# jimmyshe/liorf

Measured on AMD Instinct MI355X. Metric: LM iterations/sec (64-line scan vs 200k-pt map), higher is better.
Workload: dtype f32; 1 GPU; kitti64: 120000-pt scan vs 200000-pt local surf map, 30 LM iterations per scan (early exit off), one scan per GPU at a time, 8 distinct seeded scans in rotation, map replicated; n_q=120000, n_m=200000, distinct_scans=8, parallelism=scan-per-gpu x1

## Files before the change

### include/liorf_s2m_debug.h

```cpp
#ifndef LIORF_S2M_DEBUG_H
#define LIORF_S2M_DEBUG_H

#include "liorf_s2m.h"

#ifdef __cplusplus
extern "C" {
#endif

int  s2m_debug_device_trig(s2m_handle h, const float* x, size_t n, float* s, float* c, float* a);
int  s2m_debug_deferred(s2m_handle h, int slot);
int  s2m_time_iteration_kernel(s2m_handle h, const float pose[6], int reps, float* ms_per_launch);
int  s2m_time_iterations(s2m_handle h, const float pose[6], int reps, float* ms_per_iter, int cap);

int  s2m_time_loop_launches(s2m_handle h, const float pose[6], int reps, float* us_per_launch);

int  s2m_debug_time_steady(s2m_handle h, const float pose[6], int reps, int solve_prev, float* us_per_launch);

#define S2M_PROF_WORDS 32
int  s2m_debug_wave_profile(s2m_handle h, const float pose[6], int launches, uint64_t* out, size_t cap_waves);

int  s2m_debug_device_hypot(s2m_handle h, const float* x, const float* y, size_t n, float* r);

typedef struct s2m_debug_lm_close_out {
    float   AtA[36], AtB[6];
    int32_t n_sel_last;
    s2m_iter_trace trace;
    float   pose[6];
    float   pose_next[6];
    int32_t iters_run, converged, done, stalled, is_degenerate;
    int32_t n_rows_active;
    float   matP[36];
} s2m_debug_lm_close_out;
int  s2m_debug_lm_close(s2m_handle h, int form, int iter, const double* rows, int n_rows, const float pose0[6],
// ... 20 lines not shown
```

### liorf_amd/csrc/s2m_abi.hip

```cpp
#include <hip/hip_runtime.h>

#include <cfloat>
#include <cmath>
#include <cstdio>
#include <cstdlib>
#include <cstring>
#include <algorithm>
#include <limits>
#include <map>
#include <new>
#include <string>
#include <vector>

#include "s2m_context.hpp"
#include "s2m_kernels.hpp"

using namespace s2m;
using namespace s2m::host;

namespace {

inline uint32_t host_f2ord(float f) { uint32_t u; memcpy(&u, &f, 4); return (u & 0x80000000u) ? ~u : (u | 0x80000000u); }
inline float host_ord2f(uint32_t o) { uint32_t u = (o & 0x80000000u) ? (o & 0x7fffffffu) : ~o; float f; memcpy(&f, &u, 4); return f; }

inline float stamps_ms(const s2m_context* h, int from, int to)
{
    const unsigned long long a = h->reg.h_stamps[from], b = h->reg.h_stamps[to];
    return (b > a && h->reg.wall_clock_khz > 0) ? (float)((double)(b - a) / (double)h->reg.wall_clock_khz) : 0.0f;
}

int ensure_rows(s2m_context* h, int nblocks)
{
    const size_t rows = sizeof(double) * 2 * kAcc * (size_t)nblocks;
    int rc = ensure(h, h->reg.partials, rows + 64 + sizeof(int32_t) * 2 * (size_t)nblocks);
    if (rc) return rc;
    h->hctx.partials = h->reg.partials.as<double>();
    h->hctx.wl_count = reinterpret_cast<int32_t*>(h->reg.partials.as<unsigned char>() + rows);
// ... 229 lines not shown
}

void launch_scan_prep(hipStream_t stream, const PrepTable& t, int nslots)
{
    int npb = 0, nb = 0, ncb = 0;
    for (int k = 0; k < nslots; k++) {
        npb = std::max(npb, (int)t.s[k].npb);
        nb = std::max(nb, (t.s[k].n + 255) / 256);
        ncb = std::max(ncb, (t.s[k].n_chunks + 3) / 4);
    }
    if (npb == 0) return;
    hipLaunchKernelGGL(k_polar_count, dim3(npb, nslots), dim3(kPolarBlock), 0, stream, t);
    hipLaunchKernelGGL(k_polar_prefix, dim3(kPolarCells / 64, nslots), dim3(1024), 0, stream, t);
    hipLaunchKernelGGL(k_polar_scan, dim3(1, nslots), dim3(1024), 0, stream, t);
    hipLaunchKernelGGL(k_scatter_scan, dim3(nb, nslots), dim3(256), 0, stream, t);
    hipLaunchKernelGGL(k_chunk_parts, dim3(ncb, nslots), dim3(256), 0, stream, t);
    hipLaunchKernelGGL(k_chunk_table, dim3(1, nslots), dim3(1024), 0, stream, t);
}

}

int s2m::host::set_scan_impl(s2m_context* h, const void* pts, size_t n, size_t stride, bool on_device)
{
    S2M_HIP(h, hipSetDevice(h->device));
    PrepTable t;
    int rc = scan_slot_prepare(h, pts, n, stride, on_device, &t.s[0]);
    if (rc) return rc;
    if (n == 0) { h->reg.t_set_scan_ms = 0; h->reg.scan_timing_pending = false; return upload_ctx(h); }
    t.s[0].stamps = h->reg.h_stamps + kStampPrep0;
    launch_scan_prep(h->stream, t, 1);
    S2M_HIP(h, hipGetLastError());
    h->reg.scan_timing_pending = true;
    if (!on_device) S2M_HIP(h, hipEventSynchronize(h->reg.ev_up));
    return S2M_OK;
}

namespace {

void fill_state(s2m_context* h, DevState* s, const float pose[6])
{
    memset(s, 0, sizeof(*s));
    memcpy(s->pose, pose, 24);
    memcpy(s->pose2[0], pose, 24);
    host_pose_to_transform(pose, s->T, s->sc);
    s->T_valid = 1;
    memcpy(s->matP, h->reg.persist_matP, sizeof(s->matP));
    s->isDegenerate = h->reg.persist_degenerate;
}

int push_state(s2m_context* h, const float pose[6], unsigned long long* stamp = nullptr)
{
    DevState s;
    fill_state(h, &s, pose);
    if (h->ctx_dirty) {
        hipLaunchKernelGGL(k_set_ctx_state, dim3(1), dim3(64), 0, h->stream, h->reg.dctx.as<DevCtx>(), h->hctx, h->reg.state.as<DevState>(), s,
                           (const int32_t*)h->reg.n_waves.as<int32_t>(), stamp);
        h->ctx_dirty = false;
    } else
        hipLaunchKernelGGL(k_set_state, dim3(1), dim3(64), 0, h->stream, h->reg.state.as<DevState>(), s,
                           (const int32_t*)h->reg.n_waves.as<int32_t>(), stamp);
    S2M_HIP(h, hipGetLastError());
    return S2M_OK;
}

constexpr int kFuseMaxBlocks = 512;
static_assert(sizeof(CtxTable) <= 4096 && sizeof(StateInitTable) <= 4096 && sizeof(PrepTable) <= 4096 && sizeof(SlotTable) <= 4096,
              "kernel arguments are limited to 4 KB");

struct LoopShape {
    SlotTable tbl;
    int nslots = 1;
    int nblocks = 0;
    int table_cap = 0;
    int wpb = kBlock / 64;
    bool batch = false;
    bool split = false;
    bool late = false;
    bool split_auto = false;
    DevState* out = nullptr;
    unsigned long long* stamp = nullptr;
};

LoopShape shape_of(s2m_context* h)
{
    LoopShape sh;
    memset(&sh.tbl, 0, sizeof(sh.tbl));
    sh.tbl.ctx[0] = h->reg.dctx.as<DevCtx>();
    sh.tbl.st[0] = h->reg.state.as<DevState>();
    sh.nslots = 1; sh.nblocks = h->hctx.nblocks; sh.table_cap = h->hctx.table_cap; sh.wpb = h->hctx.wpb;
    sh.batch = h->batch.parent != nullptr && !h->batch.slot_mode;
    sh.split = h->tune.split_mode == 1;
    return sh;
}

template <bool HOOK, int NW, int MINW, int MODE, int CNW>
inline void launch_k(hipStream_t s, const LoopShape& sh, int L, int flags, int grid_x = 0)
{
    hipLaunchKernelGGL((k_register<HOOK, NW, MINW, MODE, CNW>), dim3(grid_x > 0 ? std::min(grid_x, sh.nblocks) : sh.nblocks, sh.nslots), dim3(NW * 64), 0, s,
                       sh.tbl, L, flags);
}

inline void launch_fused(s2m_context* h, const LoopShape& sh, bool hook, int L, int solve_prev)
{
// ... 22 lines not shown
}

inline void launch_certify(s2m_context* h, const LoopShape& sh, int L, int solve_prev, bool fused_loop)
{
    constexpr int NW = kBlock / 64;
    const int fl = solve_prev ? kFlagSolvePrev : 0;
    if (!fused_loop && sh.wpb == NW && h->tune.lean_certify)
        hipLaunchKernelGGL((k_certify_lean<NW, 1, kCertifyLeanWaves>), dim3(sh.nblocks, sh.nslots), dim3(NW * 64), 0, h->stream, sh.tbl, L);
    else if (sh.wpb == kBigWaves) launch_k<false, kBigWaves, kCertifyWavesBig, kCertify, kBigWaves>(h->stream, sh, L, fl);
    else                     launch_k<false, NW, kCertifyWaves, kCertify, NW>(h->stream, sh, L, fl);
}

inline void launch_iteration(s2m_context* h, const LoopShape& sh, int L, int solve_prev, bool fused_loop = true)
{
    if (!sh.split) { launch_fused(h, sh, false, L, solve_prev); return; }
    if (L == 0) { launch_search(h, sh, 0, true); return; }
    launch_certify(h, sh, L, solve_prev, fused_loop);
    launch_search(h, sh, L, false, sh.late);
}

inline void launch_finalize(s2m_context* h, const LoopShape& sh, int L, int mode, bool ends_range = false)
{
    hipLaunchKernelGGL(k_finalize, dim3(1, sh.nslots), dim3(kFinThreads), 0, h->stream, sh.tbl, L, mode,
                       ends_range ? sh.out : (DevState*)nullptr, ends_range ? sh.stamp : (unsigned long long*)nullptr);
}

inline void launch_density(s2m_context* h, const LoopShape& sh)
{
    hipLaunchKernelGGL(k_wave_density, dim3((sh.table_cap + 3) / 4, sh.nslots), dim3(256), 0, h->stream, sh.tbl, h->tune.density_raw);
    hipLaunchKernelGGL(k_chunk_table_density, dim3(1, sh.nslots), dim3(1024), 0, h->stream, sh.tbl);
}

void enqueue_loop(s2m_context* h, const LoopShape& sh_in, hipEvent_t* events, bool coarse = false, int L0 = 0, int L1 = -1)
{
    const int n = h->prm.max_iter;
    if (L1 < 0) L1 = n;
    const bool fuse = h->tune.fuse_solve && sh_in.nblocks * sh_in.nslots <= h->tune.fuse_max_blocks;
    LoopShape sh = sh_in;
    const bool split_late = sh.split_auto && !fuse && sh.wpb == kBlock / 64 && h->tune.lean_certify;
    if (h->tune.density_raw > 0 && L0 == 0) launch_density(h, sh);
    for (int L = L0; L < L1; L++) {
        const int slot = !coarse ? 2 * L : (L == 0 ? 0 : (L == 1 ? 2 : (L == n - 1 ? 6 : 4)));
        const bool open = events && (!coarse || L <= 2 || L == n - 1), close = events && (!coarse || L <= 1 || L >= n - 2);
        if (open) (void)hipEventRecord(events[slot], h->stream);
        sh.split = sh_in.split || (split_late && L >= h->tune.split_from);
        sh.late = !sh_in.split && sh.split;
        launch_iteration(h, sh, L, (fuse && L >= 2 && L != L0) ? 1 : 0, fuse);
        if (close) (void)hipEventRecord(events[slot + 1], h->stream);
        if ((!fuse || L == 0 || L == L1 - 1) && !(sh.late && h->tune.close_in_search)) launch_finalize(h, sh, L, 0, L == L1 - 1);
    }
}

int get_graph(s2m_context* h, int nblocks, int part, hipGraphExec_t* out)
{
    LoopShape sh = shape_of(h);
    sh.out = &h->reg.h_state[1];
    sh.stamp = part == 2 ? nullptr : h->reg.h_stamps + kStampLoop1;
    const long long key = (((long long)h->hctx.table_cap * 4 + part) * 256 + (part ? h->tune.seg_iters : 0)) * 4 + (sh.split ? 1 : 0) + (sh.wpb == kBigWaves ? 2 : 0);
    auto it = h->reg.graphs.find(key);
    if (it != h->reg.graphs.end()) { *out = it->second; return S2M_OK; }
    hipGraph_t graph = nullptr;
    hipGraphExec_t exec = nullptr;
    S2M_HIP(h, hipStreamBeginCapture(h->stream, hipStreamCaptureModeThreadLocal));
    enqueue_loop(h, sh, nullptr, false, part == 2 ? h->tune.seg_iters : 0, part == 1 ? h->tune.seg_iters : -1);
    hipError_t e = hipStreamEndCapture(h->stream, &graph);
    if (e != hipSuccess || !graph) return fail(h, S2M_ERR_HIP, "hipStreamEndCapture", e);
    e = hipGraphInstantiate(&exec, graph, nullptr, nullptr, 0);
    (void)hipGraphDestroy(graph);
    if (e != hipSuccess) return fail(h, S2M_ERR_HIP, "hipGraphInstantiate", e);
    h->reg.graphs[key] = exec;
    *out = exec;
    return S2M_OK;
}

int launch_loop(s2m_context* h, int part = 0)
{
    const int nblocks = h->hctx.nblocks;
    if (h->tune.use_graph) {
        hipGraphExec_t exec = nullptr;
        int rc = get_graph(h, nblocks, part, &exec);
        if (rc == S2M_OK) {
            if (part == 2) S2M_HIP(h, hipEventRecord(h->reg.ev_a2, h->stream));
            S2M_HIP(h, hipGraphLaunch(exec, h->stream));
            if (part == 2) S2M_HIP(h, hipEventRecord(h->reg.ev_b2, h->stream));
            h->hctx.density_pending = 0;
            return S2M_OK;
        }
        h->tune.use_graph = false;
    }
    LoopShape sh = shape_of(h);
    sh.stamp = part == 2 ? nullptr : h->reg.h_stamps + kStampLoop1;
    if (part == 2) S2M_HIP(h, hipEventRecord(h->reg.ev_a2, h->stream));
    enqueue_loop(h, sh, nullptr, false, part == 2 ? h->tune.seg_iters : 0, part == 1 ? h->tune.seg_iters : -1);
    S2M_HIP(h, hipGetLastError());
    if (part == 2) S2M_HIP(h, hipEventRecord(h->reg.ev_b2, h->stream));
    S2M_HIP(h, hipMemcpyAsync(&h->reg.h_state[1], h->reg.state.p, sizeof(DevState) + sizeof(s2m_iter_trace) * h->prm.max_iter, hipMemcpyDeviceToHost, h->stream));
    h->hctx.density_pending = 0;
    return S2M_OK;
}

void params_to_ctx(s2m_context* h, const s2m_params& prm)
{
    h->hctx.gate_f = nextafterf((float)prm.gate_sq, INFINITY);
    h->hctx.gate_r = nextafterf(sqrtf((float)prm.gate_sq), 0.0f);
    h->hctx.gate_sq = prm.gate_sq; h->hctx.plane_tol = prm.plane_tol; h->hctx.weight_scale = prm.weight_scale;
    h->hctx.weight_min = prm.weight_min; h->hctx.conv_deg = prm.conv_deg; h->hctx.conv_cm = prm.conv_cm;
    h->hctx.eig_thresh = prm.eig_thresh; h->hctx.min_corr = prm.min_corr; h->hctx.max_iter = prm.max_iter;
    h->hctx.early_exit = prm.early_exit;
    h->ctx_dirty = true;
}

constexpr size_t kScDesc = (size_t)S2M_SC_NUM_RING * S2M_SC_NUM_SECTOR;

int sc_reserve(s2m_context* h, size_t want)
{
    if (want <= h->sc.cap) return S2M_OK;
    size_t cap = h->sc.cap ? h->sc.cap : 256;
    while (cap < want) cap *= 2;
    struct Part { DevBuf* b; size_t elem; } parts[3] = { { &h->sc.store_desc, sizeof(double) * kScDesc },
                                                         { &h->sc.store_ring, sizeof(float) * S2M_SC_NUM_RING },
// ... 73 lines not shown
    if (hipGetDeviceCount(&count) != hipSuccess || count <= 0 || prm.device_id < 0 || prm.device_id >= count)
        return S2M_ERR_NO_DEVICE;
    if (hipSetDevice(prm.device_id) != hipSuccess) return S2M_ERR_NO_DEVICE;
    hipDeviceProp_t prop;
    if (hipGetDeviceProperties(&prop, prm.device_id) != hipSuccess) return S2M_ERR_NO_DEVICE;
    if (strncmp(prop.gcnArchName, "gfx950", 6) != 0) return S2M_ERR_NO_DEVICE;

    s2m_context* h = new (std::nothrow) s2m_context();
    if (!h) return S2M_ERR_HIP;
    h->prm = prm; h->device = prm.device_id;
    if (const char* e = getenv("S2M_NO_GRAPH")) h->tune.use_graph = !(e[0] == '1');
    if (const char* e = getenv("S2M_NO_FUSE")) h->tune.fuse_solve = !(e[0] == '1');
    if (const char* e = getenv("S2M_DENSITY_RAW")) h->tune.density_raw = atoi(e);
    if (const char* e = getenv("S2M_BIG_BLOCKS")) h->tune.big_blocks = !(e[0] == '0');
    if (const char* e = getenv("S2M_SEGMENT")) h->tune.seg_iters = atoi(e);
    if (const char* e = getenv("S2M_SPLIT")) h->tune.split_mode = atoi(e);
    if (const char* e = getenv("S2M_LOCKSTEP")) h->tune.lockstep = !(e[0] == '0');
    if (const char* e = getenv("S2M_SPLIT_FROM")) h->tune.split_from = std::max(1, atoi(e));
    if (const char* e = getenv("S2M_SEARCH_GRID")) h->tune.search_grid = std::max(1, atoi(e));
    if (const char* e = getenv("S2M_CLOSE_IN_SEARCH")) h->tune.close_in_search = (e[0] == '1');
    if (const char* e = getenv("S2M_BATCH_MINW")) h->tune.batch_minw = atoi(e);
    if (const char* e = getenv("S2M_BATCH_ENTRIES")) h->tune.batch_entries = atoi(e);
    if (const char* e = getenv("S2M_LEAN")) h->tune.lean_certify = !(e[0] == '0');
    h->tune.fuse_max_blocks = kFuseMaxBlocks;
    if (const char* e = getenv("S2M_FUSE_MAX")) h->tune.fuse_max_blocks = atoi(e);

    auto bail = [&](int code) { s2m_destroy(h); return code; };
    if (prm.stream) { h->stream = static_cast<hipStream_t>(prm.stream); h->own_stream = false; }
    else {
        if (hipStreamCreateWithFlags(&h->stream, hipStreamNonBlocking) != hipSuccess) return bail(S2M_ERR_HIP);
        h->own_stream = true;
    }
    if (hipEventCreate(&h->reg.ev_a) != hipSuccess || hipEventCreate(&h->reg.ev_b) != hipSuccess ||
        hipEventCreate(&h->reg.ev_c) != hipSuccess || hipEventCreate(&h->reg.ev_d) != hipSuccess ||
        hipEventCreate(&h->reg.ev_a2) != hipSuccess || hipEventCreate(&h->reg.ev_b2) != hipSuccess ||
        hipEventCreateWithFlags(&h->reg.ev_up, hipEventDisableTiming) != hipSuccess) return bail(S2M_ERR_HIP);
    static_assert(sizeof(DevState) % 8 == 0, "the trace follows the state block");
    if (hipHostMalloc((void**)&h->reg.h_state, sizeof(DevState) * 2 + sizeof(s2m_iter_trace) * kMaxIter) != hipSuccess) return bail(S2M_ERR_HIP);
    h->reg.h_trace = reinterpret_cast<s2m_iter_trace*>(h->reg.h_state + 2);
    if (hipHostMalloc((void**)&h->reg.h_mm, 64) != hipSuccess) return bail(S2M_ERR_HIP);
    if (hipHostMalloc((void**)&h->reg.h_stamps, sizeof(unsigned long long) * kStampCount) != hipSuccess) return bail(S2M_ERR_HIP);
    memset(h->reg.h_stamps, 0, sizeof(unsigned long long) * kStampCount);
    {
        int khz = 0;
        if (hipDeviceGetAttribute(&khz, hipDeviceAttributeWallClockRate, prm.device_id) != hipSuccess || khz <= 0) { khz = 0; (void)hipGetLastError(); }
        h->reg.wall_clock_khz = khz;
// ... 106 lines not shown
    h->reg.pending_skipped = 0;
    if (h->reg.n_m == 0) { h->reg.pending_skipped = 1; return S2M_OK; }
    if ((int)h->reg.n_q <= h->prm.min_feats) { h->reg.pending_skipped = 2; return S2M_OK; }
    int rc;
    if ((rc = push_state(h, pose, h->reg.h_stamps + kStampLoop0))) return rc;
    h->reg.seg_pending = h->prm.early_exit && h->tune.seg_iters > 1 && h->tune.seg_iters < h->prm.max_iter;
    if ((rc = launch_loop(h, h->reg.seg_pending ? 1 : 0))) return rc;
    return S2M_OK;
}

int s2m_optimize_collect(s2m_handle h, float pose[6], const s2m_imu_init* imu, s2m_result* out)
{
    if (!h || !pose) return S2M_ERR_INVALID_ARG;
    if (!h->reg.opt_pending) return fail(h, S2M_ERR_INVALID_ARG, "no optimize launch pending");
    h->reg.opt_pending = false;
    s2m_result r;
    memset(&r, 0, sizeof(r));
    r.skipped = h->reg.pending_skipped;
    h->reg.last_trace_n = 0;
    float t[6];
    memcpy(t, h->reg.pending_pose_in, 24);
    if (!r.skipped) {
        S2M_HIP(h, hipSetDevice(h->device));
        S2M_HIP(h, hipStreamSynchronize(h->stream));
        if (h->batch.parent && !h->batch.slot_mode) h->reg.t_optimize_ms = h->batch.parent->reg.t_optimize_ms;
        else h->reg.t_optimize_ms = stamps_ms(h, kStampLoop0, kStampLoop1);
        if (h->reg.seg_pending && !h->reg.h_state[1].done) {
            int rc2 = launch_loop(h, 2);
            if (rc2) return rc2;
            S2M_HIP(h, hipStreamSynchronize(h->stream));
            float t2 = 0.0f;
            S2M_HIP(h, hipEventElapsedTime(&t2, h->reg.ev_a2, h->reg.ev_b2));
            h->reg.t_optimize_ms += t2;
        }
        h->reg.seg_pending = false;
        const DevState& s = h->reg.h_state[1];
        memcpy(t, s.pose, 24);
        r.iters_run = s.iters_run; r.converged = s.converged; r.is_degenerate = s.isDegenerate;
        r.n_sel_last = s.n_sel_last;
        h->reg.persist_degenerate = s.isDegenerate;
        memcpy(h->reg.persist_matP, s.matP, sizeof(s.matP));
        int n_exec = s.iters_run, stall_at = -1;
        for (int i = 0; i < n_exec && i < kMaxIter; i++) {
            if (stall_at >= 0) { h->reg.last_trace[i] = h->reg.last_trace[stall_at]; continue; }
            h->reg.last_trace[i] = h->reg.h_trace[i];
            if (s.stalled && !h->reg.h_trace[i].stepped) stall_at = i;
        }
        h->reg.last_trace_n = n_exec < kMaxIter ? n_exec : kMaxIter;
        host_transform_update(h->prm, imu, t, r.affine);
    } else {
        host_pose_to_transform(t, r.affine, nullptr);
        r.is_degenerate = h->reg.persist_degenerate;
// ... 565 lines not shown

int s2m_debug_deferred(s2m_handle h, int slot)
{
    if (!h) return S2M_ERR_INVALID_ARG;
    if (slot >= 0) { if (slot >= (int)h->batch.kids.size()) return S2M_ERR_INVALID_ARG; h = h->batch.kids[(size_t)slot]; }
    return h->reg.h_state ? h->reg.h_state[1].deferred_total : 0;
}

int s2m_last_timing(s2m_handle h, float* optimize_ms, float* set_map_ms, float* set_scan_ms)
{
    if (!h) return S2M_ERR_INVALID_ARG;
    if (h->reg.scan_timing_pending) {
        S2M_HIP(h, hipSetDevice(h->device));
        S2M_HIP(h, hipStreamSynchronize(h->stream));
        h->reg.t_set_scan_ms = stamps_ms(h, kStampPrep0, kStampPrep1);
        h->reg.scan_timing_pending = false;
    }
    if (optimize_ms) *optimize_ms = h->reg.t_optimize_ms;
    if (set_map_ms) *set_map_ms = h->reg.t_set_map_ms;
    if (set_scan_ms) *set_scan_ms = h->reg.t_set_scan_ms;
    return S2M_OK;
}

static int time_iterations_impl(s2m_handle h, const float pose[6], int reps, float* ms_mean, float* ms_per_iter)
{
    if (!h || !pose || reps < 1) return S2M_ERR_INVALID_ARG;
    if (!h->reg.have_scan || h->reg.n_m == 0 || h->reg.n_q == 0) return fail(h, S2M_ERR_NO_SCAN, "needs a resident scan and map");
    S2M_HIP(h, hipSetDevice(h->device));
    int rc;
    if ((rc = upload_ctx(h))) return rc;
    const int nit = h->prm.max_iter;
    if (h->reg.iter_events.size() < (size_t)(2 * nit)) {
        const size_t old = h->reg.iter_events.size();
        h->reg.iter_events.resize(2 * nit);
        for (size_t k = old; k < h->reg.iter_events.size(); k++) S2M_HIP(h, hipEventCreate(&h->reg.iter_events[k]));
    }
    std::vector<double> per_iter((size_t)nit, 0.0);
    for (int rep = 0; rep < reps; rep++) {
        S2M_HIP(h, hipMemsetAsync(h->reg.cert.p, 0, sizeof(float4) * h->reg.n_q, h->stream));
        S2M_HIP(h, hipMemsetAsync(h->reg.aux.p, 0, sizeof(int4) * h->reg.n_q, h->stream));
        if ((rc = push_state(h, pose))) return rc;
        enqueue_loop(h, shape_of(h), h->reg.iter_events.data());
        h->hctx.density_pending = 0;
        S2M_HIP(h, hipGetLastError());
        S2M_HIP(h, hipStreamSynchronize(h->stream));
        for (int it = 0; it < nit; it++) {
// ... 183 lines not shown
```

### liorf_amd/csrc/s2m_context.hpp

```cpp
#pragma once
#include <hip/hip_runtime.h>

#include <cstddef>
#include <cstdint>
#include <map>
#include <string>
#include <vector>

#include "s2m_types.h"
#include "s2m_host_math.hpp"
#include "s2m_voxel.hpp"
#include "s2m_icp.hpp"
#include "s2m_project.hpp"
#include "s2m_pose_graph.hpp"

namespace s2m {
namespace host __attribute__((visibility("hidden"))) {

struct DevBuf {
    void*  p = nullptr;
    size_t cap = 0;
    DevBuf() = default;
    DevBuf(const DevBuf&) = delete;
    DevBuf& operator=(const DevBuf&) = delete;
    ~DevBuf() { (void)reset(); }
    template <typename T> T* as() const { return reinterpret_cast<T*>(p); }
    hipError_t reset(void* q = nullptr, size_t bytes = 0)
    {
        const hipError_t e = p ? hipFree(p) : hipSuccess;
        p = q; cap = bytes;
        return e;
    }
    void forget() { p = nullptr; cap = 0; }
};

constexpr size_t kDsStride = 32;

enum { kStampPrep0 = 0, kStampPrep1 = 1, kStampLoop0 = 2, kStampLoop1 = 3, kStampCount = 4 };

}
}

struct __attribute__((visibility("hidden"))) s2m_context {
    using DevBuf = s2m::host::DevBuf;

    s2m_params prm{};
    int device = 0;
    hipStream_t stream = nullptr;
    bool own_stream = false;
    std::string err;
    s2m::DevCtx hctx{};
    bool ctx_dirty = true;

    struct Registration {
        DevBuf raw_map, map_sorted, m_counts, m_cell_start, m_cell_of, m_rank_of;
        DevBuf raw_scan, qx, qy, qz, qperm, npos, front, cert, aux, plane_cache, plane_alt, npos_alt, chunk_parts, chunk_factor, wave_table, n_waves, q_counts, q_cell_start, q_cell_of, q_rank_of, q_block_hist;
        DevBuf block_sums, partials, state, dctx, mm, dbg_idx5, dbg_d2, dbg_flag, dbg_coeff, dbg_clk;
        size_t n_m = 0, n_q = 0;
        bool have_scan = false;

        s2m::DevState* h_state = nullptr;
        s2m_iter_trace* h_trace = nullptr;
        uint32_t* h_mm = nullptr;
        unsigned long long* h_stamps = nullptr;
        int wall_clock_khz = 0;

        int persist_degenerate = 0;
        float persist_matP[36] = { 0 };

        std::map<long long, hipGraphExec_t> graphs;
        std::vector<hipEvent_t> iter_events;
        hipEvent_t ev_a = nullptr, ev_b = nullptr, ev_c = nullptr, ev_d = nullptr, ev_up = nullptr;
        hipEvent_t ev_a2 = nullptr, ev_b2 = nullptr;
        float t_optimize_ms = 0, t_set_map_ms = 0, t_set_scan_ms = 0;
        int base_parts = 1;
        bool seg_pending = false;
        bool opt_pending = false;
        bool scan_timing_pending = false;
        int pending_skipped = 0;
        float pending_pose_in[6] = { 0 };
        s2m_iter_trace last_trace[s2m::kMaxIter];
        int last_trace_n = 0;
    } reg;

    struct Batch {
        s2m_context* parent = nullptr;
        std::vector<s2m_context*> kids;
        std::vector<hipStream_t> branch_streams;
        std::vector<hipEvent_t> branch_events;
        std::vector<hipEvent_t> prep_events;
        std::vector<char> prep_pending;
        hipEvent_t ev_fork = nullptr, ev_prep = nullptr;
        DevBuf kid_states;
        unsigned char* h_kid_states = nullptr;
        bool slot_mode = false;
        bool state_borrowed = false;
        std::map<std::vector<int>, hipGraphExec_t> graphs;
        std::vector<int> live;
        bool seg_pending = false;
        unsigned long long map_epoch = 0;
        unsigned long long adopted_epoch = 0;
    } batch;

    struct Tuning {
        bool use_graph = true;
        bool fuse_solve = true;
        int  fuse_max_blocks = 0;
        int  seg_iters = 8;
        int  split_mode = -1;
        bool tune_env = false;
        bool lean_certify = true;
        int  batch_entries = 1;
        int  batch_minw = 4;
        bool close_in_search = false;
        int  search_grid = 8;
        int  split_from = 8;
        bool lockstep = true;
        bool big_blocks = true;
        int  density_raw = 320;
    } tune;

    struct Voxel {
        DevBuf in, out, frames_xf, scan_ds, map_ds;
        s2m::VoxWorkspace* ws = nullptr;
        size_t scan_ds_n = 0;
        bool have_scan_ds = false;
    } voxel;

    struct ScanContext {
        DevBuf bins, out;
        DevBuf store_desc, store_ring, store_sector, cand;
        size_t n = 0, cap = 0, n_search = 0;
        int    counter = 0;
        double* h_stage = nullptr;
    } sc;

    struct KeyFrames {
        DevBuf pos, frames, tdev;
        std::vector<void*> blocks;
        size_t block_used = 0, block_cap = 0, cap = 0;
        std::vector<float> pose;
// ... 154 lines not shown
```

### liorf_amd/csrc/s2m_kernels.hpp

```cpp
#pragma once
#include <float.h>
#include <math.h>
#include <string.h>
#include "s2m_types.h"

#if defined(__HIPCC__)
#define S2M_HD __host__ __device__
#else
#define S2M_HD
#endif

namespace s2m {

template <typename T> using gptr = __attribute__((address_space(1))) T*;
template <typename T> __device__ __forceinline__ gptr<T> G(T* p) { return (gptr<T>)p; }
typedef float v4f __attribute__((ext_vector_type(4)));
typedef const __attribute__((address_space(4))) DevCtx* CtxP;
__device__ __forceinline__ CtxP ctx_const(const DevCtx* p) { return (CtxP)p; }
__device__ __forceinline__ GridDesc grid_of(CtxP cp)
{
    GridDesc g;
    g.ox = cp->g.ox; g.oy = cp->g.oy; g.oz = cp->g.oz; g.inv_e = cp->g.inv_e; g.e = cp->g.e;
    g.nx = cp->g.nx; g.ny = cp->g.ny; g.nz = cp->g.nz; g.ncells = cp->g.ncells;
    return g;
// ... 1228 lines not shown
    const float mnz = wave_min_f32(fin ? sz : INFINITY), mxz = wave_max_f32(fin ? sz : -INFINITY);
    if (!(mnx <= mxx)) return;
    const GridDesc g = grid_of(cp);
    const auto cell_start = G(cp->cell_start);
    const int bx0 = max(cell_coord(mnx, g.ox, g.inv_e, g.nx) - 1, 0), bx1 = min(cell_coord(mxx, g.ox, g.inv_e, g.nx) + 1, g.nx - 1);
    const int by0 = max(cell_coord(mny, g.oy, g.inv_e, g.ny) - 1, 0), by1 = min(cell_coord(mxy, g.oy, g.inv_e, g.ny) + 1, g.ny - 1);
    const int bz0 = max(cell_coord(mnz, g.oz, g.inv_e, g.nz) - 1, 0), bz1 = min(cell_coord(mxz, g.oz, g.inv_e, g.nz) + 1, g.nz - 1);
    const int nyb = by1 - by0 + 1, nzb = bz1 - bz0 + 1;
    if (nyb * nzb > kRowMax) return;
    int raw = 0;
    for (int r = lane; r < nyb * nzb; r += 64) {
        const int zq = r / nyb;
        const int gcell = ((bz0 + zq) * g.ny + by0 + (r - zq * nyb)) * g.nx;
        raw += cell_start[gcell + bx1 + 1] - cell_start[gcell + bx0];
    }
    raw = __builtin_amdgcn_readlane(wave_incl_scan_i32(raw), 63);
    int f = raw <= raw_limit ? 1 : (raw <= 2 * raw_limit ? 2 : (raw <= 4 * raw_limit ? 4 : 8));
    f = min(f, max(e.y / 8, 1));
    if (lane == 0 && f > 1) atomicMax(&cp->chunk_factor[e.x >> 6], f);
}

#include "s2m_register.hpp"

__device__ __forceinline__ void finalize_record_out(gptr<DevState> st, DevState* out, int max_iter, unsigned long long* stamp)
{
    static_assert(sizeof(DevState) % 4 == 0 && sizeof(s2m_iter_trace) % 4 == 0, "the record is copied word by word");
    if (out) {
        const auto src = (gptr<const uint32_t>)st;
        const auto dst = G(reinterpret_cast<uint32_t*>(out));
        const int nw = (int)((sizeof(DevState) + sizeof(s2m_iter_trace) * (size_t)max_iter) / 4);
        for (int k = threadIdx.x; k < nw; k += kFinThreads) dst[k] = src[k];
    }
    if (stamp) {
        __syncthreads();
        if (threadIdx.x == 0) *stamp = wall_clock64();
    }
}

__global__ __launch_bounds__(kFinThreads) void k_finalize(const SlotTable tbl, int iter, int mode, DevState* out, unsigned long long* stamp)
{
    const CtxP cp = ctx_const(tbl.ctx[blockIdx.y]);
    const auto st = G(tbl.st[blockIdx.y]);
    const int done0 = st->done, degen0 = st->isDegenerate;
    const int nb_act = (st->n_waves + cp->wpb - 1) / cp->wpb;
    float pose0[6];
#pragma unroll
    for (int k = 0; k < 6; k++) pose0[k] = st->pose2[iter & 1][k];
    if (mode == 0 && done0) { finalize_record_out(st, out, cp->max_iter, stamp); return; }
    __shared__ LmShared sh;
    __shared__ float s_out[8];
    if (mode == 0 && threadIdx.x == 0 && cp->wl_count) { cp->wl_count[0] = 0; cp->wl_count[1] = 0; }
    float pose[6];
    const bool ended = lm_close_iteration<kFinThreads, true>(cp, st, nb_act, iter, true, mode == 1, pose0, degen0, sh, s_out, pose);
    if (mode == 0 && !ended && threadIdx.x < 64) {
        float T[12], sc6[6];
        build_transform(pose, (int)threadIdx.x, T, sc6);
        if (threadIdx.x == 0 && !st->stalled) {
#pragma unroll
            for (int k = 0; k < 12; k++) st->T[k] = T[k];
#pragma unroll
            for (int k = 0; k < 6; k++) st->sc[k] = sc6[k];
            st->T_valid = 1;
        }
    }
    if (out || stamp) {
        __syncthreads();
        finalize_record_out(st, out, cp->max_iter, stamp);
    }
}

__global__ __launch_bounds__(256) void k_debug_sincos(const float* __restrict__ x, int n, float* __restrict__ s, float* __restrict__ c,
                                                      float* __restrict__ a)
{
    const int i = blockIdx.x * blockDim.x + threadIdx.x;
    if (i < n) { s[i] = glibc_sincosf(x[i], 0); c[i] = glibc_sincosf(x[i], 1); if (a) a[i] = glibc_atanf(x[i]); }
}

__global__ __launch_bounds__(256) void k_debug_hypot(const float* __restrict__ x, const float* __restrict__ y, int n, float* __restrict__ r)
{
    const int i = blockIdx.x * blockDim.x + threadIdx.x;
    if (i < n) r[i] = glibc_hypotf(x[i], y[i]);
}

__global__ void k_set_ctx(DevCtx* dst, DevCtx v) { if (threadIdx.x == 0 && blockIdx.x == 0) *dst = v; }
__global__ void k_set_ctx_state(DevCtx* cdst, DevCtx c, DevState* dst, DevState v, const int32_t* n_waves, unsigned long long* stamp)
{
    if (threadIdx.x == 0 && blockIdx.x == 0) { *cdst = c; v.n_waves = n_waves ? *n_waves : 0; *dst = v; if (stamp) *stamp = wall_clock64(); }
}

__global__ void k_set_ctxs(const CtxTable t) { if (threadIdx.x == 0 && t.dst[blockIdx.x]) *t.dst[blockIdx.x] = t.v[blockIdx.x]; }
// ... 280 lines not shown
```

### liorf_amd/csrc/s2m_types.h

```cpp
#pragma once
#include <stdint.h>
#include <hip/hip_runtime.h>
#include "../../include/liorf_s2m.h"
#include "../../include/liorf_s2m_debug.h"

namespace s2m {

constexpr int kBlock = 512;
constexpr int kAcc = 28;
constexpr int kFinThreads = 1024;
constexpr int kMaxIter = 64;
constexpr int kProfWords = 32;
constexpr int kBlocksQuantum = 8;
constexpr int kNbrCap = 6;
constexpr int kMaxBlocks = 512;
constexpr int kBigWaves = 16;

struct GridDesc {
    float ox, oy, oz;
    float inv_e;
    float e;
    int   nx, ny, nz;
    int   ncells;
};

struct DevState {
    float pose[6];
    float pose2[2][6];
    float T[12];
    float sc[6];
    float matP[36];
    float AtA[36];
    float AtB[6];
    int32_t isDegenerate;
    int32_t done;
    int32_t converged;
    int32_t iters_run;
    int32_t n_sel_last;
    int32_t stalled;
    int32_t n_waves;
    int32_t T_valid;
    int32_t deferred_total;
    int32_t pad_;
};

struct DevCtx {
    GridDesc g;
    const float4* map_sorted;
    const int32_t* cell_start;
    const float* qx; const float* qy; const float* qz;
    const int32_t* qperm;
    int32_t* npos;
    float4*  cert;
    int4*    aux;
    float4*  front;
    float4*  plane_cache;
    float4*  plane_alt;
    int32_t* npos_alt;
    int32_t n_q, n_m, nblocks;
    int32_t wpb;
    int32_t table_cap;
    const int2* wave_table;
    const int32_t* n_waves;
    int2*    wave_table_rw; int32_t* n_waves_rw;
    const int32_t* chunk_parts;
    int32_t* chunk_factor;
    int32_t  n_chunks;
// ... 46 lines not shown
```

### liorf_amd/s2m.py

```python
from __future__ import annotations

import ctypes as C
import importlib.util
import os
import sys

import numpy as np

_HERE = os.path.dirname(os.path.abspath(__file__))
LIB_PATH = os.environ.get("S2M_LIB") or os.path.join(_HERE, "libliorf_s2m.so")

S2M_OK = 0
S2M_ERR_CAPACITY = -5
S2M_ERR_BUSY = -6
ERRORS = {-1: "S2M_ERR_INVALID_ARG", -2: "S2M_ERR_NO_DEVICE", -3: "S2M_ERR_HIP", -4: "S2M_ERR_NO_SCAN",
          -5: "S2M_ERR_CAPACITY", -6: "S2M_ERR_BUSY"}

ABI_SYMBOLS = [
    "s2m_version", "s2m_default_params", "s2m_create", "s2m_destroy", "s2m_last_error", "s2m_set_params", "s2m_get_params",
    "s2m_set_map", "s2m_set_map_device", "s2m_set_scan", "s2m_set_scan_device",
    "s2m_optimize", "s2m_optimize_resident", "s2m_optimize_launch", "s2m_optimize_collect",
    "s2m_optimize_batch", "s2m_batch_set_scan", "s2m_batch_set_scans", "s2m_slot_set_scan", "s2m_slot_optimize_launch", "s2m_slot_optimize_collect", "s2m_optimize_batch_launch", "s2m_optimize_batch_collect", "s2m_batch_get_trace",
    "s2m_get_trace", "s2m_surf_optimization", "s2m_normal_eq", "s2m_last_timing", "s2m_debug_deferred",
    "s2m_time_iteration_kernel", "s2m_time_iterations", "s2m_make_scancontext", "s2m_debug_wave_profile", "s2m_debug_time_steady", "s2m_time_loop_launches",
    "s2m_voxel_downsample", "s2m_voxel_downsample_device", "s2m_downsample_scan", "s2m_extract_cloud",
    "s2m_transform_cloud",
    "s2m_icp_default_params", "s2m_icp_align", "s2m_debug_device_trig", "s2m_debug_device_hypot",
    "s2m_debug_lm_close", "s2m_debug_lm_close_check_args",
    "s2m_sc_reset", "s2m_sc_size", "s2m_sc_add_scan", "s2m_sc_add_descriptor", "s2m_sc_detect_loop", "s2m_sc_distance",
    "s2m_kf_default_params", "s2m_kf_reset", "s2m_kf_size", "s2m_kf_add", "s2m_kf_set_poses", "s2m_extract_surrounding",
    "s2m_loop_default_params", "s2m_loop_near_keyframes", "s2m_loop_align", "s2m_loop_closure_rs",
    "s2m_loop_align_launch", "s2m_loop_closure_rs_launch", "s2m_loop_poll", "s2m_loop_collect",
    "s2m_debug_icp_nearest", "s2m_debug_icp_time_nearest", "s2m_debug_icp_align_device", "s2m_debug_icp_tuning",
    "s2m_gmap_default_params", "s2m_global_map", "s2m_kf_map_cloud",
    "s2m_scan_layout_preset", "s2m_project_default_params", "s2m_imu_deskew_info", "s2m_project_check_args", "s2m_project_scan",
    "s2m_downsample_projected", "s2m_sc_add_projected",
    "s2m_odom_deskew_info", "s2m_project_check_args_motion", "s2m_project_scan_motion", "s2m_guess_state_init", "s2m_update_initial_guess",
    "s2m_pg_default_params", "s2m_pg_check_args", "s2m_pg_reset", "s2m_pg_size", "s2m_pg_add_prior", "s2m_pg_add_between", "s2m_pg_add_gps",
    "s2m_pg_set_initial", "s2m_pg_add_odometry", "s2m_pg_optimize", "s2m_pg_get_poses", "s2m_pg_marginal", "s2m_pg_apply_to_store",
    "s2m_pg_marginals_check_args", "s2m_pg_marginals", "s2m_pg_joint_marginal",
    "s2m_pg_optimize_launch", "s2m_pg_optimize_poll", "s2m_pg_optimize_collect", "s2m_debug_pg_rebase",
]
S2M_RING_U8, S2M_RING_U16, S2M_RING_I32 = 0, 1, 2
S2M_TIME_F32, S2M_TIME_U32_NS, S2M_TIME_U32, S2M_TIME_F64_REL = 0, 1, 2, 3
S2M_SENSOR_VELODYNE, S2M_SENSOR_LIVOX, S2M_SENSOR_OUSTER, S2M_SENSOR_MULRAN, S2M_SENSOR_ROBOSENSE = 0, 1, 2, 3, 4
S2M_IMU_QUEUE_LENGTH = 2000
# ... 164 lines not shown
    L.s2m_destroy.argtypes = [vp]
    L.s2m_set_params.argtypes = [vp, C.POINTER(Params)]
    L.s2m_get_params.argtypes = [vp, C.POINTER(Params)]
    for n in ("s2m_set_map", "s2m_set_map_device", "s2m_set_scan", "s2m_set_scan_device"):
        getattr(L, n).argtypes = [vp, vp, C.c_size_t, C.c_size_t]
    L.s2m_optimize.argtypes = [vp, vp, C.c_size_t, C.c_size_t, fp, C.POINTER(ImuInit), C.POINTER(Result)]
    L.s2m_optimize_resident.argtypes = [vp, fp, C.POINTER(ImuInit), C.POINTER(Result)]
    L.s2m_optimize_launch.argtypes = [vp, fp]
    L.s2m_optimize_collect.argtypes = [vp, fp, C.POINTER(ImuInit), C.POINTER(Result)]
    L.s2m_get_trace.argtypes = [vp, C.POINTER(IterTrace), C.c_int]
    L.s2m_optimize_batch.argtypes = [vp, C.c_int, C.POINTER(vp), C.POINTER(C.c_size_t), C.c_size_t, fp, C.POINTER(ImuInit), C.POINTER(Result)]
    L.s2m_batch_set_scan.argtypes = [vp, C.c_int, vp, C.c_size_t, C.c_size_t, C.c_int]
    L.s2m_slot_set_scan.argtypes = [vp, C.c_int, vp, C.c_size_t, C.c_size_t, C.c_int]
    L.s2m_slot_optimize_launch.argtypes = [vp, C.c_int, fp]
    L.s2m_slot_optimize_collect.argtypes = [vp, C.c_int, fp, C.POINTER(ImuInit), C.POINTER(Result)]
    L.s2m_batch_set_scans.argtypes = [vp, C.c_int, C.POINTER(C.c_void_p), C.POINTER(C.c_size_t), C.c_size_t, C.c_int]
    L.s2m_optimize_batch_launch.argtypes = [vp, C.c_int, fp]
    L.s2m_optimize_batch_collect.argtypes = [vp, C.c_int, fp, C.POINTER(ImuInit), C.POINTER(Result)]
    L.s2m_batch_get_trace.argtypes = [vp, C.c_int, C.POINTER(IterTrace), C.c_int]
    L.s2m_surf_optimization.argtypes = [vp, fp, C.POINTER(C.c_int32), fp, C.POINTER(C.c_uint8), fp]
    L.s2m_normal_eq.argtypes = [vp, fp, fp, fp, C.POINTER(C.c_int32)]
    L.s2m_last_timing.argtypes = [vp, fp, fp, fp]
    L.s2m_debug_deferred.argtypes = [vp, C.c_int]
    L.s2m_time_iteration_kernel.argtypes = [vp, fp, C.c_int, fp]
    L.s2m_time_iterations.argtypes = [vp, fp, C.c_int, fp, C.c_int]
    L.s2m_debug_wave_profile.argtypes = [vp, fp, C.c_int, C.POINTER(C.c_uint64), C.c_size_t]
    L.s2m_debug_time_steady.argtypes = [vp, fp, C.c_int, C.c_int, fp]
    L.s2m_time_loop_launches.argtypes = [vp, fp, C.c_int, fp]
    L.s2m_make_scancontext.argtypes = [vp, vp, C.c_size_t, C.c_size_t, C.POINTER(C.c_double), C.POINTER(C.c_double)]
    szp = C.POINTER(C.c_size_t)
    for n in ("s2m_voxel_downsample", "s2m_voxel_downsample_device"):
        getattr(L, n).argtypes = [vp, vp, C.c_size_t, C.c_size_t, C.c_float, vp, C.c_size_t, C.c_size_t, szp]
    L.s2m_downsample_scan.argtypes = [vp, vp, C.c_size_t, C.c_size_t, C.c_int, C.c_float, vp, C.c_size_t, C.c_size_t, szp]
    L.s2m_extract_cloud.argtypes = [vp, C.c_int, C.POINTER(vp), szp, C.c_size_t, C.c_int, fp, C.c_float,
                                    vp, C.c_size_t, C.c_size_t, szp]
    L.s2m_transform_cloud.argtypes = [vp, vp, C.c_size_t, C.c_size_t, fp, vp, C.c_size_t]
    dp, i32p = C.POINTER(C.c_double), C.POINTER(C.c_int32)
    L.s2m_debug_device_trig.argtypes = [vp, fp, C.c_size_t, fp, fp, fp]
    L.s2m_debug_device_hypot.argtypes = [vp, fp, fp, C.c_size_t, fp]
    L.s2m_debug_lm_close.argtypes = [vp, C.c_int, C.c_int, dp, C.c_int, fp, C.c_int, fp, C.POINTER(LmCloseOut)]
    L.s2m_debug_lm_close_check_args.argtypes = [C.c_int, C.c_int, C.c_int, dp, C.c_int, fp, fp, C.POINTER(LmCloseOut)]
    L.s2m_icp_default_params.argtypes = [C.POINTER(IcpParams)]
    L.s2m_icp_align.argtypes = [vp, vp, C.c_size_t, vp, C.c_size_t, C.c_size_t, C.POINTER(IcpParams), C.POINTER(IcpResult)]
    L.s2m_sc_reset.argtypes = [vp]
    L.s2m_sc_size.argtypes = [vp]
    L.s2m_sc_add_scan.argtypes = [vp, vp, C.c_size_t, C.c_size_t]
# ... 399 lines not shown
        return sn, cs, at

    def deviceHypot(self, x, y):
        a, b = np.ascontiguousarray(x, np.float32), np.ascontiguousarray(y, np.float32)
        assert a.shape == b.shape
        r = np.zeros_like(a)
        self._check(self.lib.s2m_debug_device_hypot(self.h, _fp(a), _fp(b), a.size, _fp(r)), "s2m_debug_device_hypot")
        return r

    def lmClose(self, form: int, it: int, rows, pose0, degen_in: int, matP_in) -> LmCloseOut:
        r = np.ascontiguousarray(rows, np.float64).reshape(-1, 28)
        p = np.ascontiguousarray(pose0, np.float32).reshape(6)
        m = np.ascontiguousarray(matP_in, np.float32).reshape(36)
        out = LmCloseOut()
        self._check(self.lib.s2m_debug_lm_close(self.h, form, it, r.ctypes.data_as(C.POINTER(C.c_double)), r.shape[0], _fp(p),
                                                int(degen_in), _fp(m), C.byref(out)), "s2m_debug_lm_close")
        return out

    def timing(self):
        a, b, c = C.c_float(0), C.c_float(0), C.c_float(0)
        self.lib.s2m_last_timing(self.h, C.byref(a), C.byref(b), C.byref(c))
        return dict(optimize_ms=a.value, set_map_ms=b.value, set_scan_ms=c.value)

    def time_iteration_kernel(self, pose, reps: int = 200) -> float:
        p = np.ascontiguousarray(pose, np.float32)
        ms = C.c_float(0)
        self._check(self.lib.s2m_time_iteration_kernel(self.h, _fp(p), reps, C.byref(ms)), "s2m_time_iteration_kernel")
        return ms.value

    def time_iterations(self, pose, reps: int = 10) -> np.ndarray:
        p = np.ascontiguousarray(pose, np.float32)
        out = np.zeros(64, np.float32)
        self._check(self.lib.s2m_time_iterations(self.h, _fp(p), reps, _fp(out), 64), "s2m_time_iterations")
        return out[:self.params.max_iter]

    def time_loop_launches(self, pose, reps: int = 10) -> float:
        p = np.ascontiguousarray(pose, np.float32)
        us = C.c_float(0)
        self._check(self.lib.s2m_time_loop_launches(self.h, _fp(p), reps, C.byref(us)), "s2m_time_loop_launches")
        return us.value

    def time_steady(self, pose, reps: int = 200, solve_prev: bool = True) -> float:
        p = np.ascontiguousarray(pose, np.float32)
        us = C.c_float(0)
        self._check(self.lib.s2m_debug_time_steady(self.h, _fp(p), reps, 1 if solve_prev else 0, C.byref(us)), "s2m_debug_time_steady")
        return us.value
# ... 565 lines not shown
```

Before: 53450 LM iterations/s.

## Collect LM results by spinning on a device-written ticket instead of stream sync

The finalize kernel now publishes a monotonically increasing ticket to host-visible memory with a system-scope release store after writing the result record. The host, on the graph path, spins on that word with pause instructions and falls back to hipStreamQuery and then hipStreamSynchronize, instead of always calling hipStreamSynchronize. This is meant to cut the wake-up latency of blocking stream synchronization at the end of each optimize call. The cost is a busy CPU core while waiting and extra fence work in finalize. It also adds a timing probe for set_scan prelaunch time.

```diff
diff --git a/include/liorf_s2m_debug.h b/include/liorf_s2m_debug.h
--- a/include/liorf_s2m_debug.h
+++ b/include/liorf_s2m_debug.h
@@ -9,6 +9,7 @@
 
 int  s2m_debug_device_trig(s2m_handle h, const float* x, size_t n, float* s, float* c, float* a);
 int  s2m_debug_deferred(s2m_handle h, int slot);
+int  s2m_debug_set_scan_prelaunch_us(s2m_handle h, float* us);
 int  s2m_time_iteration_kernel(s2m_handle h, const float pose[6], int reps, float* ms_per_launch);
 int  s2m_time_iterations(s2m_handle h, const float pose[6], int reps, float* ms_per_iter, int cap);
 
diff --git a/liorf_amd/csrc/s2m_abi.hip b/liorf_amd/csrc/s2m_abi.hip
--- a/liorf_amd/csrc/s2m_abi.hip
+++ b/liorf_amd/csrc/s2m_abi.hip
@@ -1,6 +1,7 @@
 #include <hip/hip_runtime.h>
 
 #include <cfloat>
+#include <chrono>
 #include <cmath>
 #include <cstdio>
 #include <cstdlib>
@@ -13,6 +14,7 @@
 #include <vector>
 
 #include "s2m_context.hpp"
+#include "s2m_ticket_wait.hpp"
 #include "s2m_kernels.hpp"
 
 using namespace s2m;
@@ -288,12 +290,14 @@
 
 int s2m::host::set_scan_impl(s2m_context* h, const void* pts, size_t n, size_t stride, bool on_device)
 {
+    const std::chrono::steady_clock::time_point t_in = std::chrono::steady_clock::now();
     S2M_HIP(h, hipSetDevice(h->device));
     PrepTable t;
     int rc = scan_slot_prepare(h, pts, n, stride, on_device, &t.s[0]);
     if (rc) return rc;
     if (n == 0) { h->reg.t_set_scan_ms = 0; h->reg.scan_timing_pending = false; return upload_ctx(h); }
     t.s[0].stamps = h->reg.h_stamps + kStampPrep0;
+    h->reg.t_prelaunch_us = std::chrono::duration<float, std::micro>(std::chrono::steady_clock::now() - t_in).count();
     launch_scan_prep(h->stream, t, 1);
     S2M_HIP(h, hipGetLastError());
     h->reg.scan_timing_pending = true;
@@ -312,6 +316,7 @@
     s->T_valid = 1;
     memcpy(s->matP, h->reg.persist_matP, sizeof(s->matP));
     s->isDegenerate = h->reg.persist_degenerate;
+    s->ticket = h->reg.ticket_count;
 }
 
 int push_state(s2m_context* h, const float pose[6], unsigned long long* stamp = nullptr)
@@ -345,6 +350,7 @@
     bool split_auto = false;
     DevState* out = nullptr;
     unsigned long long* stamp = nullptr;
+    unsigned long long* ticket = nullptr;
 };
 
 LoopShape shape_of(s2m_context* h)
@@ -413,7 +419,8 @@
 inline void launch_finalize(s2m_context* h, const LoopShape& sh, int L, int mode, bool ends_range = false)
 {
     hipLaunchKernelGGL(k_finalize, dim3(1, sh.nslots), dim3(kFinThreads), 0, h->stream, sh.tbl, L, mode,
-                       ends_range ? sh.out : (DevState*)nullptr, ends_range ? sh.stamp : (unsigned long long*)nullptr);
+                       ends_range ? sh.out : (DevState*)nullptr, ends_range ? sh.stamp : (unsigned long long*)nullptr,
+                       ends_range ? sh.ticket : (unsigned long long*)nullptr);
 }
 
 inline void launch_density(s2m_context* h, const LoopShape& sh)
@@ -447,6 +454,7 @@
     LoopShape sh = shape_of(h);
     sh.out = &h->reg.h_state[1];
     sh.stamp = part == 2 ? nullptr : h->reg.h_stamps + kStampLoop1;
+    sh.ticket = h->reg.h_stamps + kStampTicket;
     const long long key = (((long long)h->hctx.table_cap * 4 + part) * 256 + (part ? h->tune.seg_iters : 0)) * 4 + (sh.split ? 1 : 0) + (sh.wpb == kBigWaves ? 2 : 0);
     auto it = h->reg.graphs.find(key);
     if (it != h->reg.graphs.end()) { *out = it->second; return S2M_OK; }
@@ -473,6 +481,8 @@
         if (rc == S2M_OK) {
             if (part == 2) S2M_HIP(h, hipEventRecord(h->reg.ev_a2, h->stream));
             S2M_HIP(h, hipGraphLaunch(exec, h->stream));
+            h->reg.ticket_count++;
+            h->reg.ticket_wait = true;
             if (part == 2) S2M_HIP(h, hipEventRecord(h->reg.ev_b2, h->stream));
             h->hctx.density_pending = 0;
             return S2M_OK;
@@ -481,12 +491,30 @@
     }
     LoopShape sh = shape_of(h);
     sh.stamp = part == 2 ? nullptr : h->reg.h_stamps + kStampLoop1;
+    h->reg.ticket_wait = false;
     if (part == 2) S2M_HIP(h, hipEventRecord(h->reg.ev_a2, h->stream));
     enqueue_loop(h, sh, nullptr, false, part == 2 ? h->tune.seg_iters : 0, part == 1 ? h->tune.seg_iters : -1);
     S2M_HIP(h, hipGetLastError());
     if (part == 2) S2M_HIP(h, hipEventRecord(h->reg.ev_b2, h->stream));
     S2M_HIP(h, hipMemcpyAsync(&h->reg.h_state[1], h->reg.state.p, sizeof(DevState) + sizeof(s2m_iter_trace) * h->prm.max_iter, hipMemcpyDeviceToHost, h->stream));
     h->hctx.density_pending = 0;
+    return S2M_OK;
+}
+
+int await_range(s2m_context* h)
+{
+    const bool by_ticket = h->reg.ticket_wait && h->tune.collect_spin && !(h->batch.parent && !h->batch.slot_mode);
+    h->reg.ticket_wait = false;
+    if (by_ticket) {
+        int qerr = 0;
+        const int w = wait_ticket(h->reg.h_stamps + kStampTicket, h->reg.ticket_count, [h]() -> int {
+            const hipError_t e = hipStreamQuery(h->stream);
+            return e == hipSuccess ? (int)kQueryDone : (e == hipErrorNotReady ? (int)kQueryBusy : 0x10000 + (int)e);
+        }, &qerr);
+        if (w == kTicketSeen) return S2M_OK;
+        if (w == kTicketError) return fail(h, S2M_ERR_HIP, "hipStreamQuery(h->stream)", (hipError_t)(qerr - 0x10000));
+    }
+    S2M_HIP(h, hipStreamSynchronize(h->stream));
     return S2M_OK;
 }
 
@@ -606,6 +634,7 @@
     if (const char* e = getenv("S2M_BATCH_MINW")) h->tune.batch_minw = atoi(e);
     if (const char* e = getenv("S2M_BATCH_ENTRIES")) h->tune.batch_entries = atoi(e);
     if (const char* e = getenv("S2M_LEAN")) h->tune.lean_certify = !(e[0] == '0');
+    if (const char* e = getenv("S2M_COLLECT_SPIN")) h->tune.collect_spin = !(e[0] == '0');
     h->tune.fuse_max_blocks = kFuseMaxBlocks;
     if (const char* e = getenv("S2M_FUSE_MAX")) h->tune.fuse_max_blocks = atoi(e);
 
@@ -758,12 +787,18 @@
     memcpy(t, h->reg.pending_pose_in, 24);
     if (!r.skipped) {
         S2M_HIP(h, hipSetDevice(h->device));
-        S2M_HIP(h, hipStreamSynchronize(h->stream));
+        int rcw = await_range(h);
+        if (rcw) return rcw;
+        if (h->reg.scan_timing_pending && !(h->batch.parent && !h->batch.slot_mode)) {
+            h->reg.t_set_scan_ms = stamps_ms(h, kStampPrep0, kStampPrep1);
+            h->reg.scan_timing_pending = false;
+        }
         if (h->batch.parent && !h->batch.slot_mode) h->reg.t_optimize_ms = h->batch.parent->reg.t_optimize_ms;
         else h->reg.t_optimize_ms = stamps_ms(h, kStampLoop0, kStampLoop1);
         if (h->reg.seg_pending && !h->reg.h_state[1].done) {
             int rc2 = launch_loop(h, 2);
             if (rc2) return rc2;
+            h->reg.ticket_wait = false;
             S2M_HIP(h, hipStreamSynchronize(h->stream));
             float t2 = 0.0f;
             S2M_HIP(h, hipEventElapsedTime(&t2, h->reg.ev_a2, h->reg.ev_b2));
@@ -1375,6 +1410,13 @@
     return S2M_OK;
 }
 
+int s2m_debug_set_scan_prelaunch_us(s2m_handle h, float* us)
+{
+    if (!h || !us) return S2M_ERR_INVALID_ARG;
+    *us = h->reg.t_prelaunch_us;
+    return S2M_OK;
+}
+
 static int time_iterations_impl(s2m_handle h, const float pose[6], int reps, float* ms_mean, float* ms_per_iter)
 {
     if (!h || !pose || reps < 1) return S2M_ERR_INVALID_ARG;
diff --git a/liorf_amd/csrc/s2m_context.hpp b/liorf_amd/csrc/s2m_context.hpp
--- a/liorf_amd/csrc/s2m_context.hpp
+++ b/liorf_amd/csrc/s2m_context.hpp
@@ -36,7 +36,7 @@
 
 constexpr size_t kDsStride = 32;
 
-enum { kStampPrep0 = 0, kStampPrep1 = 1, kStampLoop0 = 2, kStampLoop1 = 3, kStampCount = 4 };
+enum { kStampPrep0 = 0, kStampPrep1 = 1, kStampLoop0 = 2, kStampLoop1 = 3, kStampTicket = 4, kStampCount = 5 };
 
 }
 }
@@ -75,6 +75,9 @@
         float t_optimize_ms = 0, t_set_map_ms = 0, t_set_scan_ms = 0;
         int base_parts = 1;
         bool seg_pending = false;
+        unsigned long long ticket_count = 0;
+        bool ticket_wait = false;
+        float t_prelaunch_us = 0;
         bool opt_pending = false;
         bool scan_timing_pending = false;
         int pending_skipped = 0;
@@ -117,6 +120,7 @@
         int  split_from = 8;
         bool lockstep = true;
         bool big_blocks = true;
+        bool collect_spin = true;
         int  density_raw = 320;
     } tune;
 
diff --git a/liorf_amd/csrc/s2m_kernels.hpp b/liorf_amd/csrc/s2m_kernels.hpp
--- a/liorf_amd/csrc/s2m_kernels.hpp
+++ b/liorf_amd/csrc/s2m_kernels.hpp
@@ -1274,7 +1274,8 @@
 
 #include "s2m_register.hpp"
 
-__device__ __forceinline__ void finalize_record_out(gptr<DevState> st, DevState* out, int max_iter, unsigned long long* stamp)
+__device__ __forceinline__ void finalize_record_out(gptr<DevState> st, DevState* out, int max_iter, unsigned long long* stamp,
+                                                    unsigned long long* ticket)
 {
     static_assert(sizeof(DevState) % 4 == 0 && sizeof(s2m_iter_trace) % 4 == 0, "the record is copied word by word");
     if (out) {
@@ -1283,13 +1284,23 @@
         const int nw = (int)((sizeof(DevState) + sizeof(s2m_iter_trace) * (size_t)max_iter) / 4);
         for (int k = threadIdx.x; k < nw; k += kFinThreads) dst[k] = src[k];
     }
-    if (stamp) {
+    if (ticket) {
+        __threadfence_system();
+        __syncthreads();
+        if (threadIdx.x == 0) {
+            if (stamp) __hip_atomic_store(stamp, wall_clock64(), __ATOMIC_RELEASE, __HIP_MEMORY_SCOPE_SYSTEM);
+            const unsigned long long t = st->ticket + 1;
+            st->ticket = t;
+            __hip_atomic_store(ticket, t, __ATOMIC_RELEASE, __HIP_MEMORY_SCOPE_SYSTEM);
+        }
+    } else if (stamp) {
         __syncthreads();
         if (threadIdx.x == 0) *stamp = wall_clock64();
     }
 }
 
-__global__ __launch_bounds__(kFinThreads) void k_finalize(const SlotTable tbl, int iter, int mode, DevState* out, unsigned long long* stamp)
+__global__ __launch_bounds__(kFinThreads) void k_finalize(const SlotTable tbl, int iter, int mode, DevState* out, unsigned long long* stamp,
+                                                          unsigned long long* ticket)
 {
     const CtxP cp = ctx_const(tbl.ctx[blockIdx.y]);
     const auto st = G(tbl.st[blockIdx.y]);
@@ -1298,7 +1309,7 @@
     float pose0[6];
 #pragma unroll
     for (int k = 0; k < 6; k++) pose0[k] = st->pose2[iter & 1][k];
-    if (mode == 0 && done0) { finalize_record_out(st, out, cp->max_iter, stamp); return; }
+    if (mode == 0 && done0) { finalize_record_out(st, out, cp->max_iter, stamp, ticket); return; }
     __shared__ LmShared sh;
     __shared__ float s_out[8];
     if (mode == 0 && threadIdx.x == 0 && cp->wl_count) { cp->wl_count[0] = 0; cp->wl_count[1] = 0; }
@@ -1315,9 +1326,9 @@
             st->T_valid = 1;
         }
     }
-    if (out || stamp) {
+    if (out || stamp || ticket) {
         __syncthreads();
-        finalize_record_out(st, out, cp->max_iter, stamp);
+        finalize_record_out(st, out, cp->max_iter, stamp, ticket);
     }
 }
 
diff --git a/liorf_amd/csrc/s2m_ticket_wait.hpp b/liorf_amd/csrc/s2m_ticket_wait.hpp
--- /dev/null
+++ b/liorf_amd/csrc/s2m_ticket_wait.hpp
@@ -0,0 +1,45 @@
+#pragma once
+#include <chrono>
+
+namespace s2m {
+namespace host {
+
+enum TicketQuery { kQueryDone = 0, kQueryBusy = 1 };
+enum TicketWait { kTicketSeen = 0, kTicketFallback = 1, kTicketError = 2 };
+
+inline void cpu_pause()
+{
+#if defined(__x86_64__) || defined(__i386__)
+    __builtin_ia32_pause();
+#elif defined(__aarch64__)
+    __asm__ __volatile__("yield");
+#endif
+}
+
+constexpr int kTicketPollsPerClock = 32;
+constexpr int kTicketQueryUs = 25;
+constexpr int kTicketMaxQueries = 40000;
+
+template <typename Query>
+inline int wait_ticket(const unsigned long long* word, unsigned long long expect, Query&& query, int* query_error,
+                       int query_us = kTicketQueryUs, int max_queries = kTicketMaxQueries)
+{
+    using clock = std::chrono::steady_clock;
+    for (int q = 0; q < max_queries; q++) {
+        const clock::time_point until = clock::now() + std::chrono::microseconds(query_us);
+        do {
+            for (int k = 0; k < kTicketPollsPerClock; k++) {
+                if (__atomic_load_n(word, __ATOMIC_ACQUIRE) == expect) return kTicketSeen;
+                cpu_pause();
+            }
+        } while (clock::now() < until);
+        const int st = query();
+        if (st == kQueryBusy) continue;
+        if (st != kQueryDone) { if (query_error) *query_error = st; return kTicketError; }
+        return __atomic_load_n(word, __ATOMIC_ACQUIRE) == expect ? kTicketSeen : kTicketFallback;
+    }
+    return kTicketFallback;
+}
+
+}
+}
diff --git a/liorf_amd/csrc/s2m_types.h b/liorf_amd/csrc/s2m_types.h
--- a/liorf_amd/csrc/s2m_types.h
+++ b/liorf_amd/csrc/s2m_types.h
@@ -1,4 +1,5 @@
 #pragma once
+#include <stddef.h>
 #include <stdint.h>
 #include <hip/hip_runtime.h>
 #include "../../include/liorf_s2m.h"
@@ -42,7 +43,9 @@
     int32_t T_valid;
     int32_t deferred_total;
     int32_t pad_;
+    unsigned long long ticket;
 };
+static_assert(sizeof(DevState) % 8 == 0 && offsetof(DevState, ticket) % 8 == 0, "the trace follows the state block; the ticket is one aligned 64-bit word");
 
 struct DevCtx {
     GridDesc g;
diff --git a/liorf_amd/s2m.py b/liorf_amd/s2m.py
--- a/liorf_amd/s2m.py
+++ b/liorf_amd/s2m.py
@@ -21,7 +21,7 @@
     "s2m_set_map", "s2m_set_map_device", "s2m_set_scan", "s2m_set_scan_device",
     "s2m_optimize", "s2m_optimize_resident", "s2m_optimize_launch", "s2m_optimize_collect",
     "s2m_optimize_batch", "s2m_batch_set_scan", "s2m_batch_set_scans", "s2m_slot_set_scan", "s2m_slot_optimize_launch", "s2m_slot_optimize_collect", "s2m_optimize_batch_launch", "s2m_optimize_batch_collect", "s2m_batch_get_trace",
-    "s2m_get_trace", "s2m_surf_optimization", "s2m_normal_eq", "s2m_last_timing", "s2m_debug_deferred",
+    "s2m_get_trace", "s2m_surf_optimization", "s2m_normal_eq", "s2m_last_timing", "s2m_debug_deferred", "s2m_debug_set_scan_prelaunch_us",
     "s2m_time_iteration_kernel", "s2m_time_iterations", "s2m_make_scancontext", "s2m_debug_wave_profile", "s2m_debug_time_steady", "s2m_time_loop_launches",
     "s2m_voxel_downsample", "s2m_voxel_downsample_device", "s2m_downsample_scan", "s2m_extract_cloud",
     "s2m_transform_cloud",
@@ -232,6 +232,7 @@
     L.s2m_normal_eq.argtypes = [vp, fp, fp, fp, C.POINTER(C.c_int32)]
     L.s2m_last_timing.argtypes = [vp, fp, fp, fp]
     L.s2m_debug_deferred.argtypes = [vp, C.c_int]
+    L.s2m_debug_set_scan_prelaunch_us.argtypes = [vp, fp]
     L.s2m_time_iteration_kernel.argtypes = [vp, fp, C.c_int, fp]
     L.s2m_time_iterations.argtypes = [vp, fp, C.c_int, fp, C.c_int]
     L.s2m_debug_wave_profile.argtypes = [vp, fp, C.c_int, C.POINTER(C.c_uint64), C.c_size_t]
@@ -677,6 +678,11 @@
         self.lib.s2m_last_timing(self.h, C.byref(a), C.byref(b), C.byref(c))
         return dict(optimize_ms=a.value, set_map_ms=b.value, set_scan_ms=c.value)
 
+    def set_scan_prelaunch_us(self) -> float:
+        us = C.c_float(0)
+        self._check(self.lib.s2m_debug_set_scan_prelaunch_us(self.h, C.byref(us)), "s2m_debug_set_scan_prelaunch_us")
+        return us.value
+
     def time_iteration_kernel(self, pose, reps: int = 200) -> float:
         p = np.ascontiguousarray(pose, np.float32)
         ms = C.c_float(0)
```

After: 53870 LM iterations/s, median of 2. Within noise of the previous version (+0.8%).
